# chechaohp/gan-ode

Measured on AMD Instinct MI355X. Metric: generated videos/sec (16-frame clips), higher is better.
Workload: dtype f32

## Files before the change

gan-ode_amd/_lib.py:

```python
from __future__ import annotations

import ctypes as C
import os

_HERE = os.path.dirname(os.path.abspath(__file__))
LIB_PATH = os.path.join(_HERE, "lib", "libgode.so")

i32, i64, f32, ptr = C.c_int32, C.c_int64, C.c_float, C.c_void_p
cint, u32, u64 = C.c_int, C.c_uint32, C.c_uint64

ACT_NONE, ACT_RELU, ACT_LRELU, ACT_TANH_OUT = 0, 1, 2, 3
EPI_RAW, EPI_TANH = 0, 1
FPROP, DGRAD = 0, 1
OP_IGEMM, OP_WGRAD, OP_BN_FINALIZE, OP_BN_BWD, OP_ODE_FWD, OP_ODE_BWD, OP_BCE, OP_ADAM, OP_PACK = range(1, 10)
OP_ODERNN_FWD, OP_ODERNN_BWD, OP_BN_APPLY, OP_COL2IM = 10, 11, 12, 13
OP_SDE_FWD, OP_SDE_BWD = 14, 15
OP_CDE_FWD, OP_CDE_BWD = 16, 17
OP_WGAN = 18
OP_GRU_FWD, OP_GRU_BWD = 19, 20
OP_DNOISE = 21
OP_CATEG, OP_CE = 22, 23
OP_CHSTATS, OP_CBN_EMBED, OP_CBN_EMBED_BWD, OP_CBN_APPLY, OP_CBN_BWD, OP_GRES_OUT, OP_GRES_OUT_BWD, OP_SN_FWD, OP_SN_BWD = range(24, 33)
REC_ADAM_NOISE = -1
ODE_NPARAM = 2672
ODERNN_NPARAM = 2176
SDE_NPARAM = 3216
CDE_NPARAM = 7536
CDE_MAX_N = 4096
GRU_NPARAM = 1632
SN_BWD_BLOCKS = 64


class ConvGeom(C.Structure):
    _fields_ = [(n, i32) for n in "N Ci Co Di Hi Wi Do Ho Wo kd kh kw sd sh sw pd ph pw".split()]

    def key(self):
        return tuple(getattr(self, n) for n, _ in self._fields_)


class _Op(C.Structure):
    """An op of gode_run (a GODE_OPS row of gode.h): a subclass names its kind and its `int FN(const op*, stream)` entry
    point once; _STRUCTS, the prototypes, EXPORTS and run_one's dispatch all follow from the subclasses."""


class IgemmOp(_Op):
    _fields_ = [("g", ConvGeom), ("dir", i32), ("act", i32), ("epilogue", i32), ("tile", i32), ("src", ptr),
                ("wpack", ptr), ("out", ptr), ("scale", ptr), ("shift", ptr), ("stats", ptr), ("gs", i64 * 5),
                ("work", ptr), ("groups", i32), ("pad3_", i32)]
    KIND, FN = OP_IGEMM, "gode_igemm"


class WgradOp(_Op):
    _fields_ = [("g", ConvGeom), ("act", i32), ("xform_on_y", i32), ("splits", i32), ("accumulate", i32),
                ("x", ptr), ("y", ptr), ("scale", ptr), ("shift", ptr), ("work", ptr), ("dw", ptr),
                ("co_perm", ptr), ("co_canon", i64), ("xs", i64 * 5)]
    KIND, FN = OP_WGRAD, "gode_wgrad"


class BnFinalizeOp(_Op):
    _fields_ = [("stats", ptr), ("rows", i32), ("ncols", i32), ("C", i32), ("count", i64), ("gamma", ptr),
                ("beta", ptr), ("running_mean", ptr), ("running_var", ptr), ("num_batches_tracked", ptr),
                ("mean", ptr), ("invstd", ptr), ("scale", ptr), ("shift", ptr), ("momentum", f32), ("eps", f32),
                ("training", i32), ("pad_", i32), ("groups", i32), ("rows0", i32), ("nseg", i32), ("order", i32),
                ("count1", i64), ("seg", i32 * 24), ("stats1", ptr), ("rows1", i32), ("pad3_", i32)]
    KIND, FN = OP_BN_FINALIZE, "gode_bn_finalize"


class BnBwdOp(_Op):
    _fields_ = [("g", ptr), ("y", ptr), ("M", i64), ("C", i32), ("act", i32), ("gamma", ptr), ("mean", ptr),
                ("invstd", ptr), ("scale", ptr), ("shift", ptr), ("dgamma", ptr), ("dbeta", ptr), ("work", ptr),
                ("accumulate", i32), ("eval_mode", i32), ("gin", ptr), ("groups", i32), ("pad2_", i32), ("M0", i64),
                ("r1_s", ptr), ("r1_w", ptr), ("r1_H", i32), ("r1_W", i32), ("r1_h", i32), ("r1_wd", i32), ("r1_off", i32),
                ("pad3_", i32)]
    KIND, FN = OP_BN_BWD, "gode_bn_bwd"


class OdeParams(C.Structure):
    _fields_ = [(n, ptr) for n in "Wa ba Wb bb W1 b1 W2 b2".split()]


class OdeFwdOp(_Op):
# ... 319 lines not shown
```

gan-ode_amd/csrc/conv_geom.h:

```cpp
#pragma once
#include <stdint.h>
#include "../../include/gode.h"

#if defined(__HIPCC__)
#define GODE_HD __host__ __device__ inline
#else
#define GODE_HD inline
#endif

#define GODE_MAX_PHASES 8

struct PhaseGeom {
  int32_t Md, Mh, Mw;
  int32_t M;
  int32_t Td, Th, Tw;
  int32_t K;
  int32_t Kp;
  int32_t Od, Oh, Ow;
  int32_t Pd, Ph, Pw;
  int32_t kd0, kh0, kw0;
  int32_t row0;
  int32_t img0;
  int64_t w_off;
};
// ... 80 lines not shown
  G.nphase = np;
  return 0;
}

inline int64_t gode_pack_floats(const IgemmGeom& G) {
  int64_t t = 0;
  for (int i = 0; i < G.nphase; ++i) t += (int64_t)G.Ncols * G.ph[i].Kp;
  return t;
}

GODE_HD int64_t gode_w_index(const gode_conv_geom& g, int co, int ci, int kd, int kh, int kw) {
  return ((((int64_t)co * g.Ci + ci) * g.kd + kd) * g.kh + kh) * g.kw + kw;
}

GODE_HD int64_t gode_pack_source(const gode_conv_geom& g, int dir, const IgemmGeom& G, const PhaseGeom& p, int n,
                                 int k, const int32_t* co_perm) {
  if (k >= p.K) return -1;
  int co, ci, kd, kh, kw;
  if (G.fullk) {
    const int tapn = n / g.Ci;
    ci = n - tapn * g.Ci; co = k;
    kd = tapn / (g.kh * g.kw); kh = (tapn / g.kw) % g.kh; kw = tapn % g.kw;
  } else {
    const int tap = k / G.Cg, c = k - tap * G.Cg;
    const int jw = tap % p.Tw, jh = (tap / p.Tw) % p.Th, jd = tap / (p.Tw * p.Th);
    kd = p.kd0 + jd * G.kstep_d; kh = p.kh0 + jh * G.kstep_h; kw = p.kw0 + jw * G.kstep_w;
    if (dir == GODE_FPROP) { co = n; ci = c; } else { co = c; ci = n; }
  }
  if (co_perm) { co = co_perm[co]; if (co < 0) return -1; }
  return gode_w_index(g, co, ci, kd, kh, kw);
}

GODE_HD int gode_gather_coord(int q, int S, int O, int J, int j) { return q * S + O + J * j; }
```

gan-ode_amd/csrc/igemm.hip:

```cpp
#include <stdlib.h>
#include "common.h"
#include "conv_geom.h"

int gode_launch_conv_patch_fprop(const gode_igemm_op* op, const int64_t* gs, hipStream_t st);

struct IgemmArgs {
  IgemmGeom G;
  const float* src;
  const float* w;
  float* out;
  const float* scale;
  const float* shift;
  float* stats;
  int32_t gsN, gsD, gsH, gsW, gsC;
  int32_t act, epilogue;
  int32_t MB, NB, xcd_mode;
  int32_t tapskip, dmajor;
  int32_t stagger;
  int32_t ksplit, slabs_per_split;
  float* work;
  int32_t out_numel;
  int32_t stats_rows;
  uint32_t src_bytes, w_bytes;
};

__device__ __forceinline__ void igemm_block_id(const IgemmArgs& a, int& mblk, int& nblk, int& phase, int& split) {
  const int MB = a.MB, NC = a.NB * a.G.nphase;
  split = blockIdx.x / (MB * NC);
  const int id = blockIdx.x - split * (MB * NC);
  int combo;
  if (a.xcd_mode == 1) {
    const int x = id & 7, j = id >> 3;
    if ((NC & 7) == 0) { combo = x + 8 * (j / MB); mblk = j % MB; }
    else { const int parts = 8 / NC; combo = x % NC; mblk = j * parts + x / NC; }
  } else if (a.xcd_mode == 2) {
    const int x = id & 7, j = id >> 3;
    combo = j % NC; mblk = (j / NC) * 8 + x;
  } else if (a.xcd_mode == 3) {
    const int x = id & 7, j = id >> 3;
    combo = j % NC; mblk = x * (MB >> 3) + j / NC;
  } else {
    mblk = id % MB; combo = id / MB;
  }
  nblk = combo % a.NB; phase = combo / a.NB;
}

template <int WM, int WN, int TM, int TN, bool VEC>
__global__ void __launch_bounds__(WM* WN * 64) igemm_kernel(const IgemmArgs a) {
  constexpr int NT = WM * WN * 64, BM = WM * TM * 32, BN = WN * TN * 32, LDK = 36;
  constexpr int RPP = NT / 8;
  constexpr int AP = BM / RPP, BP = BN / RPP;
  static_assert(BM % RPP == 0 && BN % RPP == 0, "tile/loader mismatch");
  constexpr int BUF = (BM + BN) * LDK;
  __shared__ __attribute__((aligned(16))) float smem[2 * BUF + BM * 5];
  int* rowinfo = reinterpret_cast<int*>(smem + 2 * BUF);
  int* outoff = rowinfo + BM * 4;

  const PhaseGeom& P = a.G.ph[blockIdx.z];
  const int mblk = blockIdx.x, nblk = blockIdx.y;
  if (mblk * BM >= P.M) return;
  const int tid = threadIdx.x, lane = tid & 63, wave = tid >> 6;
  const int wm = wave / WN, wn = wave % WN;
  const int Cg = a.G.Cg, Ncols = a.G.Ncols;
// ... 188 lines not shown
  constexpr bool DB = MODE == 1, GL = MODE >= 2, SK = MODE == 3;
  static_assert(!(GL && XF), "the LDS-DMA path cannot transform on load");
  constexpr int NT = WM * WN * 64, BM = WM * TM * 32, BN = WN * TN * 32, LDK = GL ? 32 : 36;
  constexpr int RPP = NT / 8;
  constexpr int AP = BM / RPP, BP = BN / RPP;
  static_assert(BM % RPP == 0 && BN % RPP == 0, "tile/loader mismatch");
  static_assert(!GL || RPP % 16 == 0, "swizzle key must not depend on the loader pass");
  constexpr int BUF = (BM + BN) * LDK;
  constexpr int NBUF = (DB || GL) ? 2 : 1;
  __shared__ __attribute__((aligned(16))) float smem[NBUF * BUF + BM * 5 + (MODE == 3 ? 4 + IGEMM_MAX_LIVE_TAPS : 0)];
  int* rowinfo = reinterpret_cast<int*>(smem + NBUF * BUF);
  int* outoff = rowinfo + BM * 4;
  int* tapmask = outoff + BM;
  int* taptab = tapmask + 4;

  int mblk, nblk, phase, split;
  igemm_block_id(a, mblk, nblk, phase, split);
  const PhaseGeom& P = a.G.ph[phase];
  if (mblk * BM >= P.M) return;
  if (a.stagger > 0) {
    const int q = (blockIdx.x >> 8) & 3;
    for (int i = 0; i < q * a.stagger; ++i) __builtin_amdgcn_s_sleep(64);
  }
  const int tid = threadIdx.x, lane = tid & 63, wave = tid >> 6;
  const int wm = wave / WN, wn = wave % WN;
  const int Cg = a.G.Cg, Ncols = a.G.Ncols;

  if (SK && tid < 3) tapmask[tid] = 0;
  if (SK) __syncthreads();
  for (int r = tid; r < BM; r += NT) {
    const int m = mblk * BM + r;
    int base = -1, bd = 0, bh = 0, bw = 0, oo = -1;
    if (m < P.M) {
      const int qw = m % P.Mw; int t = m / P.Mw;
      const int qh = t % P.Mh; t /= P.Mh;
      int qd, img;
      if (SK && a.dmajor > 0) { img = t % a.dmajor; qd = t / a.dmajor; }
      else { qd = t % P.Md; img = t / P.Md + P.img0; }
      base = img * a.gsN;
      bd = qd * a.G.Sd + P.Od; bh = qh * a.G.Sh + P.Oh; bw = qw * a.G.Sw + P.Ow;
      oo = (((img * a.G.Xd + qd * a.G.OSd + P.Pd) * a.G.Xh + qh * a.G.OSh + P.Ph) * a.G.Xw + qw * a.G.OSw + P.Pw) *
           Ncols;
      if (SK) {
        int md = 0, mh = 0, mw = 0;
        for (int j = 0; j < P.Td; ++j) md |= ((unsigned)(bd + a.G.J * j) < (unsigned)a.G.Gd ? 1 : 0) << j;
        for (int j = 0; j < P.Th; ++j) mh |= ((unsigned)(bh + a.G.J * j) < (unsigned)a.G.Gh ? 1 : 0) << j;
        for (int j = 0; j < P.Tw; ++j) mw |= ((unsigned)(bw + a.G.J * j) < (unsigned)a.G.Gw ? 1 : 0) << j;
        atomicOr(&tapmask[0], md); atomicOr(&tapmask[1], mh); atomicOr(&tapmask[2], mw);
      }
    }
    rowinfo[r * 4 + 0] = base; rowinfo[r * 4 + 1] = bd; rowinfo[r * 4 + 2] = bh; rowinfo[r * 4 + 3] = bw;
    outoff[r] = oo;
  }
  __syncthreads();
  if (SK) {
    if (tid == 0) {
      const int tmd = tapmask[0], tmh = tapmask[1], tmw = tapmask[2];
      int n = 0;
      for (int t = 0; t < P.Td * P.Th * P.Tw; ++t) {
        const int w_ = t % P.Tw, t2 = t / P.Tw, h_ = t2 % P.Th, d_ = t2 / P.Th;
        if (((tmd >> d_) & 1) & ((tmh >> h_) & 1) & ((tmw >> w_) & 1)) taptab[n++] = t;
      }
      tapmask[3] = n;
    }
    __syncthreads();
  }

  int rbase[AP], rbd[AP], rbh[AP], rbw[AP];
#pragma unroll
  for (int i = 0; i < AP; ++i) {
    const int r = (tid >> 3) + RPP * i;
    rbase[i] = rowinfo[r * 4 + 0]; rbd[i] = rowinfo[r * 4 + 1]; rbh[i] = rowinfo[r * 4 + 2]; rbw[i] = rowinfo[r * 4 + 3];
  }
  const int kchunk = GL ? (((tid & 7) ^ ((tid >> 4) & 7)) * 4) : (tid & 7) * 4;
  const int J = a.G.J, Gd = a.G.Gd, Gh = a.G.Gh, Gw = a.G.Gw;
  const int spt = Cg >> 5;
  const int nslab_all = SK ? __builtin_amdgcn_readfirstlane(tapmask[3]) * spt : P.K >> 5;
  const int per_split = SK ? (nslab_all + a.ksplit - 1) / a.ksplit : a.slabs_per_split;
  const int s_begin = split * per_split;
  const int s_last = a.ksplit > 1 ? (s_begin + per_split < nslab_all ? s_begin + per_split : nslab_all) : nslab_all;
// ... 644 lines not shown
      if (k > 1 && (t == TILE_256x128 || (live_taps && tiles_n >= 256))) break;
      const int64_t blocks = tiles_n * k;
      const double per_cu = (live_taps && t == TILE_128x128 && k == 1 && blocks >= 512) ? blocks / 256.0 : (double)((blocks + 255) / 256);
      const int slabs = gode_ceil_div(max_slabs, k);
      const double eff = ((per_cu >= 2 && resident >= 2) || t == TILE_256x128) ? eff2 : 0.8 * eff2;
      double cyc = per_cu * (4000.0 + slabs * cps / eff);
      if (k > 1) cyc += 2.4e9 * (2.5e-6 + (k + 1) * out_bytes / 3e12);
      if (cyc < best * 0.97) { best = cyc; best_tile = t; best_k = k; }
    }
  }
  if (cycles_out) *cycles_out = best;
  if (live_taps) {
    int64_t t128 = 0, t64 = 0;
    for (int i = 0; i < G.nphase; ++i) {
      t128 += (int64_t)gode_ceil_div(G.ph[i].M, 128) * gode_ceil_div(G.Ncols, 128);
      t64 += (int64_t)gode_ceil_div(G.ph[i].M, 64) * gode_ceil_div(G.Ncols, 64);
    }
    if (t128 < 256 && G.Ncols >= 64 && min_slabs == max_slabs) {
      int k = (int)((1152 + t64 / 2) / t64);
      if (k < 1) k = 1;
      while (k > 1 && (min_slabs / k < 8 || out_bytes * k > 192e6)) --k;
      best_tile = TILE_64x64; best_k = k;
    }
  }
  *tile_out = best_tile;
  sp_out->positions = positions;
  sp_out->ksplit = 1; sp_out->slabs_per_split = 0;
  if (best_k > 1) {
    sp_out->slabs_per_split = gode_ceil_div(max_slabs, best_k);
    sp_out->ksplit = gode_ceil_div(max_slabs, sp_out->slabs_per_split);
  }
}

static int prepare(const gode_igemm_op* op, IgemmArgs* A, int* tile, int* max_mblk, int* rows, SplitPlan* sp, int* rows0 = nullptr) {
  int rc = gode_build_igemm_geom(op->g, op->dir, &A->G);
  if (rc) return rc;
  const bool grouped = op->groups == 2;
  if (grouped) {
    if (op->dir != GODE_FPROP || op->g.N % 2 != 0 || A->G.nphase != 1) return GODE_E_ARG;
    A->G.ph[1] = A->G.ph[0];
    A->G.ph[0].M /= 2; A->G.ph[1].M = A->G.ph[0].M; A->G.ph[1].img0 = op->g.N / 2;
    A->G.nphase = 2;
  } else if (op->groups != 0 && op->groups != 1) return GODE_E_ARG;
  static const char* menv = getenv("GODE_IGEMM_MODEL");
  static const bool sweeping = getenv("GODE_IGEMM_SWEEP") != nullptr;
  const char* fenv = sweeping ? getenv("GODE_IGEMM_FORCE") : nullptr;
  int ftile = 0, fk = 0;
  if (fenv && sscanf(fenv, "%d,%d", &ftile, &fk) == 2 && op->tile == 0 && fast_geometry(A->G) && A->G.Ncols > 4 &&
      strides_allow_vec(op, A->G)) {
    int max_slabs = 0;
    for (int i = 0; i < A->G.nphase; ++i) if ((A->G.ph[i].K >> 5) > max_slabs) max_slabs = A->G.ph[i].K >> 5;
    *tile = ftile;
    sp->positions = op->g.N * A->G.Xd * A->G.Xh * A->G.Xw; sp->ksplit = 1; sp->slabs_per_split = 0;
    if (fk > 1) { sp->slabs_per_split = gode_ceil_div(max_slabs, fk); sp->ksplit = gode_ceil_div(max_slabs, sp->slabs_per_split); }
  } else if (op->tile == 0 && fast_geometry(A->G) && A->G.Ncols > 4 && strides_allow_vec(op, A->G) && (!menv || atoi(menv) != 0)) {
    choose_fast(op, A->G, tile, sp);
  } else {
  *tile = pick_tile_split_aware(op->g, A->G, op->tile);
  *sp = plan_split(op, A->G, *tile);
  }
  if (grouped && sp->ksplit > 1 && (sp->positions / 2) % SPLITK_ROWS != 0) {
    sp->ksplit = 1; sp->slabs_per_split = 0;
  }
  const int bm = tile_bm(*tile);
  int r0 = 0, mx = 0;
  for (int i = 0; i < A->G.nphase; ++i) {
    A->G.ph[i].row0 = r0;
    const int mb = gode_ceil_div(A->G.ph[i].M, bm);
    r0 += mb;
    if (mb > mx) mx = mb;
  }
  *max_mblk = mx;
  *rows = sp->ksplit > 1 ? gode_ceil_div(sp->positions, SPLITK_ROWS) : r0;
  if (rows0) *rows0 = !grouped ? *rows : (sp->ksplit > 1 ? *rows / 2 : A->G.ph[1].row0);
  return 0;
}

extern "C" int gode_igemm_stats_rows0(const gode_igemm_op* op) {
  IgemmArgs A; int tile, mx, rows, rows0; SplitPlan sp;
  int rc = prepare(op, &A, &tile, &mx, &rows, &sp, &rows0);
  return rc ? rc : rows0;
}

extern "C" double gode_igemm_model_cycles(const gode_igemm_op* op) {
  if (!op || op->groups == 2 || op->tile != 0) return -1.0;
  IgemmArgs A;
  if (gode_build_igemm_geom(op->g, op->dir, &A.G)) return -1.0;
  static const char* menv = getenv("GODE_IGEMM_MODEL");
  if (!fast_geometry(A.G) || A.G.Ncols <= 4 || !strides_allow_vec(op, A.G) || (menv && atoi(menv) == 0)) return -1.0;
  int tile; SplitPlan sp; double cyc = -1.0;
  choose_fast(op, A.G, &tile, &sp, &cyc);
  return cyc;
}

extern "C" int gode_igemm_stats_segments(const gode_igemm_op* op, int32_t split_images, int32_t* seg) {
  if (!op || !seg || op->groups == 2 || split_images <= 0 || split_images >= op->g.N) return GODE_E_ARG;
  IgemmArgs A; int tile, mx, rows; SplitPlan sp;
  int rc = prepare(op, &A, &tile, &mx, &rows, &sp);
  if (rc) return rc;
  if (sp.ksplit > 1) {
    const int64_t per_img = (int64_t)A.G.Xd * A.G.Xh * A.G.Xw;
    const int64_t b = (int64_t)split_images * per_img;
    if (b % SPLITK_ROWS != 0) return GODE_E_SHAPE;
    seg[0] = 0; seg[1] = (int32_t)(b / SPLITK_ROWS); seg[2] = rows;
    return 1;
  }
  const int bm = tile_bm(tile);
  for (int i = 0; i < A.G.nphase; ++i) {
    const PhaseGeom& P = A.G.ph[i];
    const int64_t per_img = (int64_t)P.Md * P.Mh * P.Mw;
    const int64_t b = (int64_t)split_images * per_img;
    if (P.M != (int64_t)op->g.N * per_img) return GODE_E_SHAPE;
    if (b % bm != 0) return GODE_E_SHAPE;
    seg[3 * i] = P.row0; seg[3 * i + 1] = P.row0 + (int32_t)(b / bm); seg[3 * i + 2] = P.row0 + gode_ceil_div(P.M, bm);
  }
  return A.G.nphase;
}

extern "C" int gode_igemm_stats_rows(const gode_igemm_op* op) {
  IgemmArgs A; int tile, mx, rows; SplitPlan sp;
  int rc = prepare(op, &A, &tile, &mx, &rows, &sp);
  return rc ? rc : rows;
}

extern "C" int64_t gode_igemm_work_size(const gode_igemm_op* op) {
  IgemmArgs A; int tile, mx, rows; SplitPlan sp;
  int rc = prepare(op, &A, &tile, &mx, &rows, &sp);
  if (rc) return rc;
  return sp.ksplit > 1 ? (int64_t)sp.ksplit * sp.positions * A.G.Ncols : 0;
}

template <int WM, int WN, int TM, int TN>
static int launch(IgemmArgs& A, bool vec, int max_mblk, bool double_buf, const SplitPlan& sp, hipStream_t st) {
  constexpr int BN = WN * TN * 32;
  dim3 grid(max_mblk, gode_ceil_div(A.G.Ncols, BN), A.G.nphase), block(WM * WN * 64);
  static const bool generic_forced = getenv("GODE_IGEMM_GENERIC") != nullptr;
  bool fast = vec && fast_geometry(A.G) && (sp.ksplit > 1 || !generic_forced);
  if (sp.ksplit > 1 && (!fast || A.work == nullptr)) return GODE_E_ARG;
  A.ksplit = sp.ksplit; A.slabs_per_split = sp.slabs_per_split;
  if (fast) {
    const int MB = max_mblk, NB = (int)grid.y, NC = NB * A.G.nphase;
    A.MB = MB; A.NB = NB; A.xcd_mode = 0;
    static const char* senv = getenv("GODE_IGEMM_STAGGER");
    A.stagger = senv ? atoi(senv) : 0;
#ifndef GODE_ABLATION_BUILD
    if (A.stagger < 0) A.stagger = 0;
#endif
    static const char* xenv = getenv("GODE_IGEMM_XCD");
    const int force = xenv ? atoi(xenv) : -1;
    const int64_t wbytes = gode_pack_floats(A.G) * 4;
    const bool ok1 = (NC % 8 == 0) || (NC < 8 && 8 % NC == 0 && MB % (8 / NC) == 0);
    const bool ok2 = MB % 8 == 0;
    const int64_t images = (int64_t)A.out_numel / ((int64_t)A.G.Xd * A.G.Xh * A.G.Xw * A.G.Ncols);
    const int64_t in_bytes = images * A.G.Gd * A.G.Gh * A.G.Gw * A.G.Cg * 4;
    int mode = ok2 ? (wbytes * 8 < 3 * in_bytes ? 3 : 0) : 0;
    if (A.dmajor > 0) mode = ok2 ? 2 : (ok1 ? 1 : 0);
    if (force == 0) mode = 0;
    if (force == 1 && ok1) mode = 1;
    if (force == 2 && ok2) mode = 2;
    if (force == 3 && ok2) mode = 3;
    A.xcd_mode = mode;
    dim3 g1(MB * NC * sp.ksplit);
    const bool has_xf = A.scale != nullptr || A.act != GODE_ACT_NONE;
    static const char* genv = getenv("GODE_IGEMM_GLDS");
    const bool glds = (genv ? atoi(genv) != 0 : true) && A.src_bytes != 0 && A.w_bytes != 0;
    if (!has_xf && glds && !double_buf) {
      if (A.tapskip) hipLaunchKernelGGL((igemm_fast_kernel<WM, WN, TM, TN, 3, false>), g1, block, 0, st, A);
      else hipLaunchKernelGGL((igemm_fast_kernel<WM, WN, TM, TN, 2, false>), g1, block, 0, st, A);
    } else if (double_buf) {
      if (has_xf) hipLaunchKernelGGL((igemm_fast_kernel<WM, WN, TM, TN, 1, true>), g1, block, 0, st, A);
      else hipLaunchKernelGGL((igemm_fast_kernel<WM, WN, TM, TN, 1, false>), g1, block, 0, st, A);
    } else {
      if (has_xf) hipLaunchKernelGGL((igemm_fast_kernel<WM, WN, TM, TN, 0, true>), g1, block, 0, st, A);
      else hipLaunchKernelGGL((igemm_fast_kernel<WM, WN, TM, TN, 0, false>), g1, block, 0, st, A);
    }
    if (sp.ksplit > 1) {
      GODE_LAUNCH_CHECK();
      if (A.G.Ncols % 4 == 0 && ((uintptr_t)A.work % 16) == 0 && ((uintptr_t)A.out % 16) == 0)
        hipLaunchKernelGGL(igemm_splitk_reduce_vec_kernel, dim3(gode_ceil_div(sp.positions, SPLITK_ROWS), gode_ceil_div(A.G.Ncols, 64)),
                           dim3(256), 0, st, A.work, A.out, A.stats, sp.positions, A.G.Ncols, sp.ksplit, A.epilogue);
      else
        hipLaunchKernelGGL(igemm_splitk_reduce_kernel, dim3(gode_ceil_div(sp.positions, SPLITK_ROWS)), dim3(256), 0, st, A.work, A.out,
                           A.stats, sp.positions, A.G.Ncols, sp.ksplit, A.epilogue);
    }
  }
  else if (vec) hipLaunchKernelGGL((igemm_kernel<WM, WN, TM, TN, true>), grid, block, 0, st, A);
  else hipLaunchKernelGGL((igemm_kernel<WM, WN, TM, TN, false>), grid, block, 0, st, A);
  GODE_LAUNCH_CHECK();
  return 0;
}

extern "C" int gode_igemm(const gode_igemm_op* op, void* stream) {
  if (!op || !op->src || !op->wpack || !op->out) return GODE_E_ARG;
  IgemmArgs A;
  int tile, max_mblk, rows;
  SplitPlan sp;
  int rc = prepare(op, &A, &tile, &max_mblk, &rows, &sp);
  if (rc) return rc;
  if (max_mblk == 0) return 0;
  const IgemmGeom& G = A.G;
  int64_t gs[5];
  if (gode_strides_are_channels_last(op->gs)) {
    gs[4] = 1; gs[3] = G.Cg; gs[2] = (int64_t)G.Gw * gs[3]; gs[1] = (int64_t)G.Gh * gs[2]; gs[0] = (int64_t)G.Gd * gs[1];
  } else {
    for (int i = 0; i < 5; ++i) gs[i] = op->gs[i];
  }
  int64_t span = 1 + (int64_t)(op->g.N - 1) * gs[0] + (int64_t)(G.Gd - 1) * gs[1] + (int64_t)(G.Gh - 1) * gs[2] +
                 (int64_t)(G.Gw - 1) * gs[3] + (int64_t)(G.Cg - 1) * gs[4];
  int64_t outn = (int64_t)op->g.N * G.Xd * G.Xh * G.Xw * G.Ncols;
  for (int i = 0; i < 5; ++i) if (gs[i] < 0) return GODE_E_ARG;
  if (span >= (1ll << 31) || outn >= (1ll << 31)) return GODE_E_SHAPE;
  if (op->src && op->wpack && op->out && ((uintptr_t)op->wpack % 16) == 0) {
    const int pr = gode_launch_conv_patch_fprop(op, gs, (hipStream_t)stream);
    if (pr != 0) return pr < 0 ? pr : 0;
  }
  A.src = op->src; A.w = op->wpack; A.out = op->out; A.scale = op->scale; A.shift = op->shift; A.stats = op->stats;
  A.gsN = (int)gs[0]; A.gsD = (int)gs[1]; A.gsH = (int)gs[2]; A.gsW = (int)gs[3]; A.gsC = (int)gs[4];
  A.act = op->act; A.epilogue = op->epilogue;
  A.stagger = 0;
  A.dmajor = 0;
  A.tapskip = igemm_wants_tapskip(op, G);
  if (A.tapskip) A.dmajor = op->g.N;
  A.stats_rows = rows;
  A.src_bytes = span * 4 < (1ll << 31) ? (uint32_t)(span * 4) : 0u;
  A.w_bytes = gode_pack_floats(G) * 4 < (1ll << 31) ? (uint32_t)(gode_pack_floats(G) * 4) : 0u;
  A.work = op->work; A.out_numel = (int32_t)outn; A.ksplit = 1; A.slabs_per_split = 0; A.MB = 0; A.NB = 0; A.xcd_mode = 0;
  if ((op->scale == nullptr) != (op->shift == nullptr)) return GODE_E_ARG;
  const bool vec = gs[4] == 1 && (G.Cg % 4) == 0 && (gs[0] % 4) == 0 && (gs[1] % 4) == 0 && (gs[2] % 4) == 0 &&
                   (gs[3] % 4) == 0 && ((uintptr_t)op->src % 16) == 0 &&
                   (op->scale == nullptr || ((uintptr_t)op->scale % 16 == 0 && (uintptr_t)op->shift % 16 == 0));
  if (((uintptr_t)op->wpack % 16) != 0) return GODE_E_ARG;
  hipStream_t st = (hipStream_t)stream;
  if (op->groups != 2) {
    int maxM = 0, minK = 1 << 30; bool kp_ok = true;
    for (int i = 0; i < G.nphase; ++i) {
      if (G.ph[i].M > maxM) maxM = G.ph[i].M;
      if (G.ph[i].K < minK) minK = G.ph[i].K;
      kp_ok = kp_ok && G.ph[i].Kp == G.ph[i].K;
    }
    const int lpp = G.Cg / 4;
    int maxK = 0;
    for (int i = 0; i < G.nphase; ++i) if (G.ph[i].Kp > maxK) maxK = G.ph[i].Kp;
    const bool one_tap = G.nphase == 1 && G.ph[0].K == G.Cg;
    if (vec && kp_ok && G.Ncols <= 4 && G.Ncols * maxK <= PW_MAXW && op->stats == nullptr && op->tile == 0 &&
        maxM >= (one_tap ? 4096 : 65536) && (lpp == 4 || lpp == 8 || lpp == 16 || lpp == 32 || lpp == 64)) {
      PwArgs D; D.a = A; D.lpp = lpp;
      for (int i = 0; i < G.nphase; ++i) {
        D.dMw[i] = make_fastdiv((uint32_t)G.ph[i].Mw); D.dMh[i] = make_fastdiv((uint32_t)G.ph[i].Mh);
        D.dMd[i] = make_fastdiv((uint32_t)G.ph[i].Md);
      }
      int64_t blocks = ((int64_t)maxM + (64 / lpp) * 4 * 8 - 1) / ((64 / lpp) * 4 * 8);
      if (blocks > (one_tap ? 4096 : 2048)) blocks = one_tap ? 4096 : 2048;
      if (one_tap) hipLaunchKernelGGL(conv_pointwise_kernel<true>, dim3((int)blocks, 1), dim3(256), 0, st, D);
      else hipLaunchKernelGGL(conv_pointwise_kernel<false>, dim3((int)blocks, G.nphase), dim3(256), 0, st, D);
      GODE_LAUNCH_CHECK();
// ... 214 lines not shown
```

gan-ode_amd/engine.py:

```python
from __future__ import annotations

import ctypes as C
from dataclasses import dataclass
from typing import List, Optional, Sequence

import numpy as np
import torch

from . import _lib as L


def make_geom(N, Ci, Co, xi, yo, k, s, p) -> L.ConvGeom:
    return L.ConvGeom(N, Ci, Co, xi[0], xi[1], xi[2], yo[0], yo[1], yo[2], k[0], k[1], k[2], s[0], s[1], s[2],
                      p[0], p[1], p[2])


def conv_out(i, k, s, p):
    return (i + 2 * p - k) // s + 1


def dptr(t: Optional[torch.Tensor]):
    return None if t is None else t.data_ptr()


# ... 54 lines not shown
        self._G2 = groups == 2 or self.split > 0
        self._last_parts = False
        if groups not in (1, 2) or (groups == 2 and (owns_input or specs[0].fwd_dir != L.FPROP or specs[0].has_bn
                                                     or specs[0].geom.N % 2)):
            raise ValueError("grouped ConvStack: two groups, Conv stack, caller-owned input, no BatchNorm on layer 0")
        self.nl = len(specs)
        self.noisy = any(s.noise for s in specs)
        if self.noisy and (owns_input or self.split):
            raise ValueError("instance noise: caller-owned input, no split stack")
        self.momentum, self.eps = momentum, eps
        self.busy = False
        self.generation = 0
        self._fwd_training = True
        self.pack_cache = pack_cache if pack_cache is not None else {}
        lib = L.lib()
        f32 = dict(dtype=torch.float32, device=device)
        self.x_in = torch.zeros(specs[0].in_dims(), **f32) if owns_input else None
        self.x0n = torch.empty(specs[0].in_dims(), **f32) if specs[0].noise else None
        self.y = [torch.empty(s.out_dims(), **f32) for s in specs[:-1]]
        self.a = [torch.empty(s.out_dims(), **f32) if self._materialize(l) else None for l, s in enumerate(specs[:-1])]
        self.out_dims = specs[-1].out_dims()
        self.wpack_f, self.wpack_b = [], [None] * self.nl
        self.stats, self.stat_rows = [], []
        self.mean, self.invstd, self.scale, self.shift = [], [], [], []
        self._two_f, self._two_b, self._rows_ab = {}, {}, {}
        for l, s in enumerate(specs):
            n = lib.gode_pack_size(C.byref(s.geom), s.fwd_dir)
            if n <= 0:
                raise RuntimeError(f"bad geometry for pack ({n})")
            self.wpack_f.append(self._shared_pack(l, s.fwd_dir, n))
            C_out = s.out_dims()[4]
            two = self._two_f[l] = bool(self.split) and 0 < l < self.nl - 1 and self._two_launches(s.geom, s.fwd_dir)
            if s.has_bn:
                probe = L.IgemmOp(g=s.geom, dir=s.fwd_dir, tile=0, groups=groups)
                if two:
                    ra, rb = (lib.gode_igemm_stats_rows(C.byref(L.IgemmOp(g=self._part_geom(s.geom, n), dir=s.fwd_dir, tile=0)))
                              for n in (self.split, s.geom.N - self.split))
                    rows = ra + rb if ra > 0 and rb > 0 else -1
                    self._rows_ab[l] = (ra, rb)
                else:
                    rows = lib.gode_igemm_stats_rows(C.byref(probe))
                if rows <= 0:
                    raise RuntimeError(f"layer {l}: no partial-statistics layout for this geometry ({rows})")
                ncols = self._ncols(s)
                self.stat_rows.append(rows)
                self.stats.append(torch.empty(rows * 2 * ncols, **f32))
                ng = 2 if self._G2 else 1
                self.mean.append(torch.empty(ng * C_out, **f32)); self.invstd.append(torch.empty(ng * C_out, **f32))
                self.scale.append(torch.empty(ng * C_out, **f32)); self.shift.append(torch.empty(ng * C_out, **f32))
                if self.split and not two:
                    seg = (C.c_int32 * 24)()
                    nseg = lib.gode_igemm_stats_segments(C.byref(probe), self.split, seg)
                    if nseg <= 0:
                        raise ValueError(f"layer {l}: the statistics rows do not split at image {self.split} ({nseg})")
                    self.__dict__.setdefault("_segs", {})[l] = (nseg, list(seg))
            else:
                self.stat_rows.append(0); self.stats.append(None)
                self.mean.append(None); self.invstd.append(None); self.scale.append(None); self.shift.append(None)
        self._ig_work = None
        self._fwd = {}
        self._bwd = {}
        self.g = None
        self._param_ptrs = None

    def _shared_pack(self, l, direction, n):
        key = ("buf", l, direction)
        buf = self.pack_cache.get(key)
# ... 55 lines not shown

    def _head_as_gemm(self, l):
        s = self.specs[l]
        g = s.geom
        taps = g.kh * g.kw
        pixels = g.N * g.Ho * g.Wo
        if (l != self.nl - 1 or self.groups != 1 or s.fwd_dir != L.DGRAD or s.has_bn or g.kd != 1 or g.Di != 1 or g.Do != 1
                or g.Ci > 4 or taps == 1 or taps * g.Ci <= 4 or g.Co % 32 != 0 or pixels < 16384
                or (g.Ho == 1 and g.Wo == 1) or s.epilogue not in (L.EPI_RAW, L.EPI_TANH)):
            return None
        return make_geom(pixels, g.Ci, g.Co, (1, g.kh, g.kw), (1, 1, 1), (1, g.kh, g.kw), (1, 1, 1), (0, 0, 0))

    def _tail_as_gemm(self):
        s = self.specs[0]
        g = s.geom
        taps = g.kd * g.kh * g.kw
        pos = g.N * g.Do * g.Ho * g.Wo
        if (self.groups != 1 or s.fwd_dir != L.FPROP or g.Ci > 4 or taps * g.Ci < 64 or g.Co % 32 != 0 or pos < 16384 or
                g.Di != (g.Do - 1) * g.sd - 2 * g.pd + g.kd or g.Hi != (g.Ho - 1) * g.sh - 2 * g.ph + g.kh or
                g.Wi != (g.Wo - 1) * g.sw - 2 * g.pw + g.kw):
            return None
        return make_geom(pos, g.Ci, g.Co, (g.kd, g.kh, g.kw), (1, 1, 1), (g.kd, g.kh, g.kw), (1, 1, 1), (0, 0, 0))

    def _in_src(self, l):
        if l == 0:
            return self.x0n if self.x0n is not None else self.x_in
        return self.a[l - 1] if self.a[l - 1] is not None else self.y[l - 1]

    def _in_xform(self, l):
        if l == 0 or self.a[l - 1] is not None:
            return None, None, L.ACT_NONE
        s = self.specs[l - 1]
        return (self.scale[l - 1], self.shift[l - 1], s.act) if s.has_bn else (None, None, s.act)

    def _count(self, l):
        d = self.specs[l].out_dims()
        return d[0] * d[1] * d[2] * d[3]

    def param_ptrs(self):
        out = []
        for p in self.params:
            for t in (p.weight, p.gamma, p.beta, p.running_mean, p.running_var, p.num_batches_tracked):
                out.append(None if t is None else t.data_ptr())
        return tuple(out)

    def _refresh(self):
        ptrs = self.param_ptrs()
        if ptrs != self._param_ptrs:
            self._fwd, self._bwd, self._param_ptrs = {}, {}, ptrs
            self._all_igemm = []

    def invalidate_packs(self):
        for k in [k for k in self.pack_cache if k[0] == "ver"]:
            del self.pack_cache[k]

    def weights_key(self):
        return tuple((p.weight._version, getattr(p.weight, "_gode_ver", 0)) for p in self.params)

    @staticmethod
    def _part_geom(g, n):
        h = L.ConvGeom(*g.key())
        h.N = n
        return h

    def _two_launches(self, g, direction):
        lib = L.lib()
# ... 77 lines not shown
                                         out=dptr(self._head_cols), scale=dptr(sc), shift=dptr(sh)))
                c2i = L.Col2imOp(cols=dptr(self._head_cols), out=None, N=g.N, Hi=g.Ho, Wi=g.Wo, Ho=g.Hi, Wo=g.Wi, C=g.Ci,
                                 kh=g.kh, kw=g.kw, sh=g.sh, sw=g.sw, ph=g.ph, pw=g.pw, epilogue=s.epilogue)
                ops.append(c2i)
                patch["last"] = c2i
                if l == 0:
                    raise RuntimeError("a one-layer stack cannot use the GEMM + col2im head")
                continue
            want_stats = s.has_bn and training
            if self._last_parts and l == self.nl - 1:
                per_in, per_out, Cs = int(np.prod(s.in_dims()[1:])), int(np.prod(s.out_dims()[1:])), sc.numel() // 2
                pair = []
                for n, img0, k in ((self.split, 0, 0), (s.geom.N - self.split, self.split, 1)):
                    pair.append(L.IgemmOp(g=self._part_geom(s.geom, n), dir=s.fwd_dir, act=act, epilogue=s.epilogue, tile=0,
                                          src=src.data_ptr() + 4 * img0 * per_in, wpack=dptr(self.wpack_f[l]), out=None,
                                          scale=sc.data_ptr() + 4 * Cs * k, shift=sh.data_ptr() + 4 * Cs * k))
                ops += pair
                patch["last"], patch["last2"] = pair[0], (pair[1], 4 * self.split * per_out)
                continue
            if self._two_f.get(l):
                ra = self._rows_ab[l][0] if s.has_bn else 0
                per_in, per_out = int(np.prod(s.in_dims()[1:])), int(np.prod(s.out_dims()[1:]))
                for n, img0, st_off in ((self.split, 0, 0), (s.geom.N - self.split, self.split, ra * 2 * self._ncols(s))):
                    ops.append(L.IgemmOp(g=self._part_geom(s.geom, n), dir=s.fwd_dir, act=act, epilogue=s.epilogue, tile=0,
                                         src=src.data_ptr() + 4 * img0 * per_in, wpack=dptr(self.wpack_f[l]),
                                         out=self.y[l].data_ptr() + 4 * img0 * per_out, scale=dptr(sc), shift=dptr(sh),
                                         stats=self.stats[l].data_ptr() + 4 * st_off if want_stats else None, groups=0))
                op = None
            else:
                op = L.IgemmOp(g=s.geom, dir=s.fwd_dir, act=act, epilogue=s.epilogue, tile=0, src=dptr(src),
                               wpack=dptr(self.wpack_f[l]), out=dptr(self.y[l]) if l < self.nl - 1 else None,
                               scale=dptr(sc), shift=dptr(sh),
                               stats=dptr(self.stats[l]) if want_stats else None,
                               groups=2 if (G2 and s.has_bn) else 0)
                ops.append(op)
            if l == 0:
                patch["first"] = op
            if l == self.nl - 1:
                patch["last"] = op
            if s.has_bn:
                rows0 = lib.gode_igemm_stats_rows0(C.byref(op)) if G2 else 0
                fin = L.BnFinalizeOp(stats=dptr(self.stats[l]), rows=self.stat_rows[l], ncols=self._ncols(s),
                                     C=s.out_dims()[4], count=self._count(l) // self.groups, gamma=dptr(p.gamma),
                                     beta=dptr(p.beta), running_mean=dptr(p.running_mean),
                                     running_var=dptr(p.running_var),
                                     num_batches_tracked=dptr(p.num_batches_tracked), mean=dptr(self.mean[l]),
                                     invstd=dptr(self.invstd[l]), scale=dptr(self.scale[l]),
                                     shift=dptr(self.shift[l]), momentum=self.momentum, eps=self.eps,
                                     training=1 if training else 0, groups=self.groups if G2 else 0, rows0=rows0)
                if self.split:
                    per_img = self._count(l) // s.geom.N
                    fin.groups, fin.order = 2, self.split_order
                    fin.count, fin.count1 = per_img * self.split, per_img * (s.geom.N - self.split)
                    if self._two_f.get(l):
                        ra, rb = self._rows_ab[l]
                        fin.rows, fin.rows1 = ra, rb
                        fin.stats1 = self.stats[l].data_ptr() + 4 * ra * 2 * self._ncols(s)
                    else:
                        nseg, seg = self._segs[l]
                        fin.nseg = nseg
                        for k in range(3 * nseg):
                            fin.seg[k] = seg[k]
                ops.append(fin)
            if l < self.nl - 1 and self.a[l] is not None:
                d = s.out_dims()
                M = d[0] * d[1] * d[2] * d[3]
                M0 = M // 2 if (G2 and s.has_bn) else ((M // d[0]) * self.split if (self.split and s.has_bn) else 0)
# ... 326 lines not shown
```

include/gode.h:

```cpp
#ifndef GODE_H
#define GODE_H
#include <stdint.h>
#ifdef __cplusplus
extern "C" {
#endif

#define GODE_VERSION 105

enum { GODE_OK = 0, GODE_E_ARG = -1, GODE_E_SHAPE = -2, GODE_E_KIND = -3 };
enum { GODE_ACT_NONE = 0, GODE_ACT_RELU = 1, GODE_ACT_LRELU = 2,
       GODE_ACT_TANH_OUT = 3  };
enum { GODE_EPI_RAW = 0, GODE_EPI_TANH = 1 };
enum { GODE_FPROP = 0, GODE_DGRAD = 1 };

typedef struct gode_conv_geom {
  int32_t N, Ci, Co;
  int32_t Di, Hi, Wi;
  int32_t Do, Ho, Wo;
  int32_t kd, kh, kw;
  int32_t sd, sh, sw;
  int32_t pd, ph, pw;
} gode_conv_geom;

typedef struct gode_igemm_op {
  gode_conv_geom g;
  int32_t dir, act, epilogue, tile;
  const float* src;
  const float* wpack;
  float* out;
  const float* scale;
  const float* shift;
  float* stats;
  int64_t gs[5];
  float* work;
  int32_t groups, pad3_;
} gode_igemm_op;
int gode_igemm(const gode_igemm_op* op, void* stream);
int64_t gode_igemm_work_size(const gode_igemm_op* op);
int gode_igemm_stats_rows(const gode_igemm_op* op);
int gode_igemm_stats_rows0(const gode_igemm_op* op);
int gode_igemm_stats_segments(const gode_igemm_op* op, int32_t split_images, int32_t* seg);
double gode_igemm_model_cycles(const gode_igemm_op* op);
int64_t gode_pack_size(const gode_conv_geom* g, int dir);
int gode_pack_weights(const gode_conv_geom* g, int dir, const float* w, float* wpack, const int32_t* co_perm,
                      int32_t co_canon, void* stream);

typedef struct gode_wgrad_op {
  gode_conv_geom g;
  int32_t act, xform_on_y, splits, accumulate;
  const float* x;
  const float* y;
  const float* scale;
  const float* shift;
  float* work;
  float* dw;
  const int32_t* co_perm; int64_t co_canon;
  int64_t xs[5];
} gode_wgrad_op;
int gode_wgrad(const gode_wgrad_op* op, void* stream);
int64_t gode_wgrad_work_size(const gode_wgrad_op* op);
int gode_wgrad_auto_splits(const gode_conv_geom* g);

typedef struct gode_bn_finalize_op {
  const float* stats; int32_t rows, ncols, C; int64_t count;
  const float* gamma; const float* beta;
  float* running_mean; float* running_var; int64_t* num_batches_tracked;
  float* mean; float* invstd; float* scale; float* shift;
  float momentum, eps; int32_t training, pad_;
// ... 329 lines not shown
```

Measured before the change: 35350.

## Add 2D tap-skipping for stride-2 transposed convs with boundary-class block ordering

Result: faster. 36350 (median of 6 runs) (+2.8%).

```diff
diff --git a/gan-ode_amd/_lib.py b/gan-ode_amd/_lib.py
--- a/gan-ode_amd/_lib.py
+++ b/gan-ode_amd/_lib.py
@@ -46,7 +46,7 @@
 class IgemmOp(_Op):
     _fields_ = [("g", ConvGeom), ("dir", i32), ("act", i32), ("epilogue", i32), ("tile", i32), ("src", ptr),
                 ("wpack", ptr), ("out", ptr), ("scale", ptr), ("shift", ptr), ("stats", ptr), ("gs", i64 * 5),
-                ("work", ptr), ("groups", i32), ("pad3_", i32)]
+                ("work", ptr), ("groups", i32), ("tapskip", i32)]
     KIND, FN = OP_IGEMM, "gode_igemm"
 
 
diff --git a/gan-ode_amd/csrc/conv_geom.h b/gan-ode_amd/csrc/conv_geom.h
--- a/gan-ode_amd/csrc/conv_geom.h
+++ b/gan-ode_amd/csrc/conv_geom.h
@@ -136,3 +136,61 @@
 }
 
 GODE_HD int gode_gather_coord(int q, int S, int O, int J, int j) { return q * S + O + J * j; }
+
+GODE_HD int gode_live_tap_mask(int q, int S, int O, int J, int T, int Gx) {
+  int m = 0;
+  for (int j = 0; j < T; ++j) m |= ((unsigned)gode_gather_coord(q, S, O, J, j) < (unsigned)Gx ? 1 : 0) << j;
+  return m;
+}
+
+GODE_HD void gode_pmajor_row(const PhaseGeom& P, int N, int m, int* img, int* qd, int* qh, int* qw) {
+  const int pos = m / N;
+  *img = m - pos * N;
+  *qw = pos % P.Mw; const int t = pos / P.Mw;
+  *qh = t % P.Mh; *qd = t / P.Mh;
+}
+
+struct TapOrder {
+  int32_t on, mper, Mh, Mw;
+  int32_t short0_h, short0_w;
+};
+
+GODE_HD void gode_taporder_decode(const TapOrder& o, int NB, int nphase, int id, int* mblk, int* nblk, int* phase) {
+  const int A = o.Mh - 1, B = o.Mw - 1, NC = NB * nphase;
+  const int c0 = A * B * NC * o.mper, c1 = c0 + B * NC * o.mper, c2 = c1 + A * NC * o.mper;
+  int r, n, cls;
+  if (id < c0) { r = id; n = A * B; cls = 0; }
+  else if (id < c1) { r = id - c0; n = B; cls = 1; }
+  else if (id < c2) { r = id - c1; n = A; cls = 2; }
+  else { r = id - c2; n = 1; cls = 3; }
+  const int combo = r / (n * o.mper), rr = r - combo * (n * o.mper);
+  const int pos = rr / o.mper, msub = rr - pos * o.mper;
+  int h, w;
+  if (cls == 0) { h = pos / B; w = pos - h * B; }
+  else if (cls == 1) { h = A; w = pos; }
+  else if (cls == 2) { h = pos; w = B; }
+  else { h = A; w = B; }
+  *phase = combo / NB; *nblk = combo - *phase * NB;
+  const int qh = ((o.short0_h >> *phase) & 1) ? (h + 1 == o.Mh ? 0 : h + 1) : h;
+  const int qw = ((o.short0_w >> *phase) & 1) ? (w + 1 == o.Mw ? 0 : w + 1) : w;
+  *mblk = (qh * o.Mw + qw) * o.mper + msub;
+}
+
+inline int gode_taporder_build(const IgemmGeom& G, int N, int bm, TapOrder* o) {
+  o->on = 0; o->mper = 0; o->Mh = o->Mw = 0; o->short0_h = o->short0_w = 0;
+  if (N % bm != 0 || G.nphase < 1) return 0;
+  for (int i = 0; i < G.nphase; ++i) {
+    const PhaseGeom& P = G.ph[i];
+    if (P.Md != 1 || P.Td != 1 || P.Mh != G.ph[0].Mh || P.Mw != G.ph[0].Mw || P.Mh < 2 || P.Mw < 2) return 0;
+    for (int dim = 0; dim < 2; ++dim) {
+      const int M = dim ? P.Mw : P.Mh, T = dim ? P.Tw : P.Th, O = dim ? P.Ow : P.Oh, S = dim ? G.Sw : G.Sh, Gx = dim ? G.Gw : G.Gh;
+      const int full = (1 << T) - 1;
+      int nshort = 0, where = -1;
+      for (int q = 0; q < M; ++q) if (gode_live_tap_mask(q, S, O, G.J, T, Gx) != full) { ++nshort; where = q; }
+      if (nshort != 1 || (where != 0 && where != M - 1)) return 0;
+      if (where == 0) { if (dim) o->short0_w |= 1 << i; else o->short0_h |= 1 << i; }
+    }
+  }
+  o->on = 1; o->mper = N / bm; o->Mh = G.ph[0].Mh; o->Mw = G.ph[0].Mw;
+  return 1;
+}
diff --git a/gan-ode_amd/csrc/igemm.hip b/gan-ode_amd/csrc/igemm.hip
--- a/gan-ode_amd/csrc/igemm.hip
+++ b/gan-ode_amd/csrc/igemm.hip
@@ -16,6 +16,8 @@
   int32_t act, epilogue;
   int32_t MB, NB, xcd_mode;
   int32_t tapskip, dmajor;
+  int32_t pmajor;
+  TapOrder ord;
   int32_t stagger;
   int32_t ksplit, slabs_per_split;
   float* work;
@@ -29,6 +31,7 @@
   split = blockIdx.x / (MB * NC);
   const int id = blockIdx.x - split * (MB * NC);
   int combo;
+  if (a.ord.on) { gode_taporder_decode(a.ord, a.NB, a.G.nphase, id, &mblk, &nblk, &phase); return; }
   if (a.xcd_mode == 1) {
     const int x = id & 7, j = id >> 3;
     if ((NC & 7) == 0) { combo = x + 8 * (j / MB); mblk = j % MB; }
@@ -283,20 +286,20 @@
     const int m = mblk * BM + r;
     int base = -1, bd = 0, bh = 0, bw = 0, oo = -1;
     if (m < P.M) {
-      const int qw = m % P.Mw; int t = m / P.Mw;
-      const int qh = t % P.Mh; t /= P.Mh;
+      int qw = m % P.Mw; int t = m / P.Mw;
+      int qh = t % P.Mh; t /= P.Mh;
       int qd, img;
       if (SK && a.dmajor > 0) { img = t % a.dmajor; qd = t / a.dmajor; }
+      else if (SK && a.pmajor > 0) gode_pmajor_row(P, a.pmajor, m, &img, &qd, &qh, &qw);
       else { qd = t % P.Md; img = t / P.Md + P.img0; }
       base = img * a.gsN;
       bd = qd * a.G.Sd + P.Od; bh = qh * a.G.Sh + P.Oh; bw = qw * a.G.Sw + P.Ow;
       oo = (((img * a.G.Xd + qd * a.G.OSd + P.Pd) * a.G.Xh + qh * a.G.OSh + P.Ph) * a.G.Xw + qw * a.G.OSw + P.Pw) *
            Ncols;
       if (SK) {
-        int md = 0, mh = 0, mw = 0;
-        for (int j = 0; j < P.Td; ++j) md |= ((unsigned)(bd + a.G.J * j) < (unsigned)a.G.Gd ? 1 : 0) << j;
-        for (int j = 0; j < P.Th; ++j) mh |= ((unsigned)(bh + a.G.J * j) < (unsigned)a.G.Gh ? 1 : 0) << j;
-        for (int j = 0; j < P.Tw; ++j) mw |= ((unsigned)(bw + a.G.J * j) < (unsigned)a.G.Gw ? 1 : 0) << j;
+        const int md = gode_live_tap_mask(qd, a.G.Sd, P.Od, a.G.J, P.Td, a.G.Gd);
+        const int mh = gode_live_tap_mask(qh, a.G.Sh, P.Oh, a.G.J, P.Th, a.G.Gh);
+        const int mw = gode_live_tap_mask(qw, a.G.Sw, P.Ow, a.G.J, P.Tw, a.G.Gw);
         atomicOr(&tapmask[0], md); atomicOr(&tapmask[1], mh); atomicOr(&tapmask[2], mw);
       }
     }
@@ -1007,9 +1010,84 @@
   }
 }
 
+static bool tapskip2d_eligible(const gode_igemm_op* op, const IgemmGeom& G) {
+  if (op->tapskip < 1 || op->dir != GODE_DGRAD || op->groups == 2 || G.fullk || op->scale != nullptr || op->act != GODE_ACT_NONE)
+    return false;
+  if (op->g.sd != 1 || op->g.sh != 2 || op->g.sw != 2) return false;
+  for (int i = 0; i < G.nphase; ++i) {
+    const PhaseGeom& P = G.ph[i];
+    if (P.Md != 1 || P.Td != 1 || P.Th * P.Tw <= 1 || P.Th * P.Tw >= IGEMM_MAX_LIVE_TAPS || P.M != G.ph[0].M) return false;
+  }
+  return true;
+}
+
+static double model_tapskip2d(const gode_igemm_op* op, const IgemmGeom& G, bool forced, int* tile_out) {
+  static const int tiles[4] = {TILE_128x128, TILE_128x64, TILE_64x64, TILE_128x32};
+  const int N = op->g.N, spt = G.Cg >> 5;
+  double best = 1e300; *tile_out = 0;
+  for (int ti = 0; ti < 4; ++ti) {
+    const int t = tiles[ti], bm = tile_bm(t), bn = tile_bn(t);
+    if (bn >= 2 * G.Ncols && bn > 32) continue;
+    if (t == TILE_128x32 && G.Ncols > 32) continue;
+    TapOrder o;
+    const bool ordered = gode_taporder_build(G, N, bm, &o) != 0;
+    if (!ordered && !forced) continue;
+    const double cps = t == TILE_128x128 ? 4096.0 : (t == TILE_128x64 ? 2048.0 : 1024.0);
+    const int resident = t == TILE_128x128 ? 2 : (t == TILE_128x64 ? 3 : 4);
+    const double eff = t == TILE_64x64 ? 0.70 : (t == TILE_128x32 ? 0.62 : 0.76);
+    const int nb = gode_ceil_div(G.Ncols, bn);
+    double total = 0, cmin = 1e300, cmax = 0; int64_t nmax = 0, ntiles = 0;
+    for (int i = 0; i < G.nphase; ++i) {
+      const PhaseGeom& P = G.ph[i];
+      const int64_t per_pos = (int64_t)gode_ceil_div(N, bm) * nb;
+      for (int qh = 0; qh < P.Mh; ++qh) {
+        const int lh = __builtin_popcount(gode_live_tap_mask(qh, G.Sh, P.Oh, G.J, P.Th, G.Gh));
+        for (int qw = 0; qw < P.Mw; ++qw) {
+          const int lw = __builtin_popcount(gode_live_tap_mask(qw, G.Sw, P.Ow, G.J, P.Tw, G.Gw));
+          const double c = 4000.0 + lh * lw * (1800.0 + spt * cps / eff);
+          total += c * per_pos; ntiles += per_pos;
+          if (c < cmin) cmin = c;
+          if (c > cmax) { cmax = c; nmax = 0; }
+          if (c == cmax) nmax += per_pos;
+        }
+      }
+    }
+    double cyc;
+    if (ordered && ntiles > 256 * (int64_t)resident) {
+      cyc = total / 256.0 + cmin;
+      const double floor_ = (double)((nmax + 255) / 256) * cmax;
+      if (cyc < floor_) cyc = floor_;
+    } else {
+      cyc = (double)((ntiles + 255) / 256) * cmax;
+      if (forced && !ordered) cyc = total / 256.0 + cmax;
+    }
+    if (cyc < best) { best = cyc; *tile_out = t; }
+  }
+  return best;
+}
+
+static int igemm_force_env(int* ftile, int* fk, int* fskip) {
+  static const bool sweeping = getenv("GODE_IGEMM_SWEEP") != nullptr;
+  const char* fenv = sweeping ? getenv("GODE_IGEMM_FORCE") : nullptr;
+  *ftile = 0; *fk = 0; *fskip = -1;
+  const int nf = fenv ? sscanf(fenv, "%d,%d,%d", ftile, fk, fskip) : 0;
+  if (nf < 3) *fskip = -1;
+  return nf;
+}
+
+static bool take_tapskip2d(const gode_igemm_op* op, const IgemmGeom& G, const SplitPlan& sp, double cycles, int fskip, int* t2,
+                           double* c2) {
+  *t2 = 0; *c2 = -1.0;
+  if (!tapskip2d_eligible(op, G) || sp.ksplit > 1 || fskip == 0) return false;
+  const bool forced = fskip == 1 || op->tapskip >= 2;
+  *c2 = model_tapskip2d(op, G, forced, t2);
+  return *t2 != 0 && (forced || (cycles > 0 && *c2 < 0.97 * cycles));
+}
+
 static int prepare(const gode_igemm_op* op, IgemmArgs* A, int* tile, int* max_mblk, int* rows, SplitPlan* sp, int* rows0 = nullptr) {
   int rc = gode_build_igemm_geom(op->g, op->dir, &A->G);
   if (rc) return rc;
+  A->tapskip = 0; A->dmajor = 0; A->pmajor = 0; A->ord.on = 0;
   const bool grouped = op->groups == 2;
   if (grouped) {
     if (op->dir != GODE_FPROP || op->g.N % 2 != 0 || A->G.nphase != 1) return GODE_E_ARG;
@@ -1018,21 +1096,30 @@
     A->G.nphase = 2;
   } else if (op->groups != 0 && op->groups != 1) return GODE_E_ARG;
   static const char* menv = getenv("GODE_IGEMM_MODEL");
-  static const bool sweeping = getenv("GODE_IGEMM_SWEEP") != nullptr;
-  const char* fenv = sweeping ? getenv("GODE_IGEMM_FORCE") : nullptr;
-  int ftile = 0, fk = 0;
-  if (fenv && sscanf(fenv, "%d,%d", &ftile, &fk) == 2 && op->tile == 0 && fast_geometry(A->G) && A->G.Ncols > 4 &&
-      strides_allow_vec(op, A->G)) {
+  int ftile, fk, fskip;
+  const int nf = igemm_force_env(&ftile, &fk, &fskip);
+  const bool modelled = op->tile == 0 && fast_geometry(A->G) && A->G.Ncols > 4 && strides_allow_vec(op, A->G);
+  double cycles = -1.0;
+  if (nf >= 2 && ftile > 0 && modelled) {
     int max_slabs = 0;
     for (int i = 0; i < A->G.nphase; ++i) if ((A->G.ph[i].K >> 5) > max_slabs) max_slabs = A->G.ph[i].K >> 5;
     *tile = ftile;
     sp->positions = op->g.N * A->G.Xd * A->G.Xh * A->G.Xw; sp->ksplit = 1; sp->slabs_per_split = 0;
     if (fk > 1) { sp->slabs_per_split = gode_ceil_div(max_slabs, fk); sp->ksplit = gode_ceil_div(max_slabs, sp->slabs_per_split); }
-  } else if (op->tile == 0 && fast_geometry(A->G) && A->G.Ncols > 4 && strides_allow_vec(op, A->G) && (!menv || atoi(menv) != 0)) {
-    choose_fast(op, A->G, tile, sp);
+  } else if (modelled && (!menv || atoi(menv) != 0)) {
+    choose_fast(op, A->G, tile, sp, &cycles);
   } else {
   *tile = pick_tile_split_aware(op->g, A->G, op->tile);
   *sp = plan_split(op, A->G, *tile);
+  }
+  if (igemm_wants_tapskip(op, A->G)) { A->tapskip = 1; A->dmajor = op->g.N; }
+  else if (modelled) {
+    int t2; double c2;
+    if (take_tapskip2d(op, A->G, *sp, cycles, fskip, &t2, &c2)) {
+      if (!(nf >= 2 && ftile > 0)) *tile = t2;
+      A->tapskip = 1; A->pmajor = op->g.N;
+      gode_taporder_build(A->G, op->g.N, tile_bm(*tile), &A->ord);
+    }
   }
   if (grouped && sp->ksplit > 1 && (sp->positions / 2) % SPLITK_ROWS != 0) {
     sp->ksplit = 1; sp->slabs_per_split = 0;
@@ -1065,6 +1152,9 @@
   if (!fast_geometry(A.G) || A.G.Ncols <= 4 || !strides_allow_vec(op, A.G) || (menv && atoi(menv) == 0)) return -1.0;
   int tile; SplitPlan sp; double cyc = -1.0;
   choose_fast(op, A.G, &tile, &sp, &cyc);
+  int ftile, fk, fskip, t2; double c2;
+  igemm_force_env(&ftile, &fk, &fskip);
+  if (!igemm_wants_tapskip(op, A.G) && take_tapskip2d(op, A.G, sp, cyc, fskip, &t2, &c2)) cyc = c2;
   return cyc;
 }
 
@@ -1073,6 +1163,7 @@
   IgemmArgs A; int tile, mx, rows; SplitPlan sp;
   int rc = prepare(op, &A, &tile, &mx, &rows, &sp);
   if (rc) return rc;
+  if (A.pmajor > 0) return GODE_E_SHAPE;
   if (sp.ksplit > 1) {
     const int64_t per_img = (int64_t)A.G.Xd * A.G.Xh * A.G.Xw;
     const int64_t b = (int64_t)split_images * per_img;
@@ -1130,15 +1221,18 @@
     const int64_t in_bytes = images * A.G.Gd * A.G.Gh * A.G.Gw * A.G.Cg * 4;
     int mode = ok2 ? (wbytes * 8 < 3 * in_bytes ? 3 : 0) : 0;
     if (A.dmajor > 0) mode = ok2 ? 2 : (ok1 ? 1 : 0);
+    if (A.pmajor > 0) mode = 0;
     if (force == 0) mode = 0;
     if (force == 1 && ok1) mode = 1;
     if (force == 2 && ok2) mode = 2;
     if (force == 3 && ok2) mode = 3;
     A.xcd_mode = mode;
+    if (A.ord.on && MB != A.ord.Mh * A.ord.Mw * A.ord.mper) A.ord.on = 0;
     dim3 g1(MB * NC * sp.ksplit);
     const bool has_xf = A.scale != nullptr || A.act != GODE_ACT_NONE;
     static const char* genv = getenv("GODE_IGEMM_GLDS");
     const bool glds = (genv ? atoi(genv) != 0 : true) && A.src_bytes != 0 && A.w_bytes != 0;
+    if (!(A.tapskip && !has_xf && glds && !double_buf)) A.ord.on = 0;
     if (!has_xf && glds && !double_buf) {
       if (A.tapskip) hipLaunchKernelGGL((igemm_fast_kernel<WM, WN, TM, TN, 3, false>), g1, block, 0, st, A);
       else hipLaunchKernelGGL((igemm_fast_kernel<WM, WN, TM, TN, 2, false>), g1, block, 0, st, A);
@@ -1193,9 +1287,6 @@
   A.gsN = (int)gs[0]; A.gsD = (int)gs[1]; A.gsH = (int)gs[2]; A.gsW = (int)gs[3]; A.gsC = (int)gs[4];
   A.act = op->act; A.epilogue = op->epilogue;
   A.stagger = 0;
-  A.dmajor = 0;
-  A.tapskip = igemm_wants_tapskip(op, G);
-  if (A.tapskip) A.dmajor = op->g.N;
   A.stats_rows = rows;
   A.src_bytes = span * 4 < (1ll << 31) ? (uint32_t)(span * 4) : 0u;
   A.w_bytes = gode_pack_floats(G) * 4 < (1ll << 31) ? (uint32_t)(gode_pack_floats(G) * 4) : 0u;
diff --git a/gan-ode_amd/engine.py b/gan-ode_amd/engine.py
--- a/gan-ode_amd/engine.py
+++ b/gan-ode_amd/engine.py
@@ -110,7 +110,7 @@
             C_out = s.out_dims()[4]
             two = self._two_f[l] = bool(self.split) and 0 < l < self.nl - 1 and self._two_launches(s.geom, s.fwd_dir)
             if s.has_bn:
-                probe = L.IgemmOp(g=s.geom, dir=s.fwd_dir, tile=0, groups=groups)
+                probe = L.IgemmOp(g=s.geom, dir=s.fwd_dir, tile=0, groups=groups, tapskip=self._tapskip(l))
                 if two:
                     ra, rb = (lib.gode_igemm_stats_rows(C.byref(L.IgemmOp(g=self._part_geom(s.geom, n), dir=s.fwd_dir, tile=0)))
                               for n in (self.split, s.geom.N - self.split))
@@ -232,6 +232,10 @@
             return None, None, L.ACT_NONE
         s = self.specs[l - 1]
         return (self.scale[l - 1], self.shift[l - 1], s.act) if s.has_bn else (None, None, s.act)
+
+    def _tapskip(self, l):
+        s = self.specs[l]
+        return int(s.fwd_dir == L.DGRAD and not self._G2 and self._in_xform(l) == (None, None, L.ACT_NONE))
 
     def _count(self, l):
         d = self.specs[l].out_dims()
@@ -375,7 +379,7 @@
                                wpack=dptr(self.wpack_f[l]), out=dptr(self.y[l]) if l < self.nl - 1 else None,
                                scale=dptr(sc), shift=dptr(sh),
                                stats=dptr(self.stats[l]) if want_stats else None,
-                               groups=2 if (G2 and s.has_bn) else 0)
+                               groups=2 if (G2 and s.has_bn) else 0, tapskip=self._tapskip(l))
                 ops.append(op)
             if l == 0:
                 patch["first"] = op
diff --git a/include/gode.h b/include/gode.h
--- a/include/gode.h
+++ b/include/gode.h
@@ -33,7 +33,8 @@
   float* stats;
   int64_t gs[5];
   float* work;
-  int32_t groups, pad3_;
+  int32_t groups;
+  int32_t tapskip;
 } gode_igemm_op;
 int gode_igemm(const gode_igemm_op* op, void* stream);
 int64_t gode_igemm_work_size(const gode_igemm_op* op);
```
